# MarkTakken/kf2vecFSW

Hardware: AMD Instinct MI355X
Metric: Gbases/s k-mer→.kf build at k=7; achieved HBM GB/s vs gfx950 peak (higher is better)
Workload: dtype u32

## Files before the change

kf2vecfsw_amd/csrc/kf_bucket.hip:

```cpp
#include <hip/hip_runtime.h>
#include <stdint.h>
#include <stdlib.h>

#include <algorithm>
#include <cstdio>
#include <mutex>
#include <vector>

#include "kf_front.h"
#include "kf_internal.h"

namespace kf {


constexpr int kBkWaves = 16;
constexpr int kBkBits = 15;
constexpr uint64_t kPieceMax = (8ull << 20) - (64ull << 10);
constexpr uint32_t kBkLagShift = 3;
constexpr uint32_t kBkSlots = 2;
constexpr uint32_t kBkRoundWeights = 0x060B1114;
constexpr int kBkGroupWindows = 4;
constexpr bool bk_pre2(int K) { return K <= 10; }
constexpr uint32_t bk_rl(int K) { return K == 10 ? 4 : 0; }

// ... 858 lines not shown
        double sum[8] = {0, 0, 0, 0, 0, 0, 0, 0};
        for (int i = 0; i < grid; ++i)
            for (int x = 0; x < 8; ++x) sum[x] += (double)prof_h[8 * i + x];
        const double np = sum[2] > 0 ? sum[2] : 1;
        int occ = 0;
        (void)hipOccupancyMaxActiveBlocksPerMultiprocessor(&occ, (const void*)fn, waves * kWave, lds);
        fprintf(stderr, "[kf_bucket k=%d] grid %d x %d waves, LDS %u B, resident workgroups per CU %d\n", k, grid,
                waves, lds, occ);
        fprintf(stderr, "[kf_bucket k=%d] pieces %.0f cycles/piece: phase1 %.3g phase2 %.3g "
                "(records %.3g, barrier %.3g, flush %.3g, barrier %.3g)\n",
                k, sum[2], sum[0] / np, sum[1] / np, sum[3] / np, sum[4] / np, sum[5] / np, sum[6] / np);
        fprintf(stderr, "[kf_bucket k=%d] per wave, cycles per piece:", k);
        for (int w = 0; w < waves; ++w) {
            double v[4] = {0, 0, 0, 0};
            for (int i = 0; i < grid; ++i)
                for (int x = 0; x < 4; ++x) v[x] += (double)prof_h[8 * grid + 4 * (waves * i + w) + x];
            fprintf(stderr, "\n  w%d records %.3g (consume %.3g) barrier %.3g | phase-1 barrier %.3g", w, v[0] / np,
                    v[3] / np, v[1] / np, v[2] / np);
        }
        fprintf(stderr, "\n");
    }
    return KF_OK;
}

}

extern "C" int kf_workspace_release(void) {
    int dev = 0;
    if (hipGetDevice(&dev) != hipSuccess) return kf_fail(KF_EHIP, "hipGetDevice failed");
    if (dev < 0 || dev >= 64) return kf_fail(KF_EINVAL, "device index out of range");
    std::lock_guard<std::mutex> lk(g_mu);
    DevState& d = g_dev[dev];
    if (hipDeviceSynchronize() != hipSuccess) return kf_fail(KF_EHIP, "hipDeviceSynchronize failed");
    for (int k = 0; k <= KF_MAX_K; ++k) {
        if (d.col_idx[k]) (void)hipFree(d.col_idx[k]);
        if (d.bcol[k]) (void)hipFree(d.bcol[k]);
        d.col_idx[k] = nullptr;
        d.bcol[k] = nullptr;
    }
    if (d.scratch) (void)hipFree(d.scratch);
    if (d.pstart) (void)hipFree(d.pstart);
    d.scratch = nullptr;
    d.scratch_bytes = 0;
    d.pstart = nullptr;
    d.pstart_n = 0;
    return KF_OK;
}
```

kf2vecfsw_amd/csrc/kf_count.hip:

```cpp
#include <hip/hip_runtime.h>
#include <stdint.h>
#include <stdlib.h>

#include <mutex>

#include "kf_front.h"
#include "kf_internal.h"

namespace kf {

constexpr int kBlock = 1024;
constexpr uint32_t kWaveWeights = 20u | 17u << 8 | 11u << 16 | 6u << 24;
constexpr int kXRing = 2;

__device__ __forceinline__ void wg_span(const CountArgs& A, uint64_t& lo, uint64_t& hi) {
    const uint64_t base = A.goff[0];
    const uint64_t total = A.goff[A.n_genomes] - base;
    const uint64_t G = gridDim.x, b = blockIdx.x;
    lo = base + ((total / G * b + (total % G) * b / G) & ~(uint64_t)15);
    hi = (b + 1 == G) ? base + total : base + ((total / G * (b + 1) + (total % G) * (b + 1) / G) & ~(uint64_t)15);
}

template <int K>
struct XL {
    static constexpr uint32_t P = K >= 8 ? (1u << 17) : (2u << (2 * (K + 1)));
    static constexpr uint32_t S = K >= 8 ? (1u << 15) : (2u << (2 * K));
    static constexpr uint32_t bytes = P + S;
};
constexpr int kXChunk = 3 * kChunk;
static_assert((uint32_t)kXChunk == kLattice, "wave ranges are split on the iteration lattice (split_at_lattice)");
constexpr uint32_t kLatticeMaxIters = 2560;
constexpr uint32_t kHot7 = 0xC000C000u, kStep7 = 0x4000u;
constexpr uint32_t kHot8 = 0xE000E000u, kStep8 = 0x2000u;
constexpr uint32_t kHot6 = 0x80008000u, kStep6 = 0x8000u;
template <int K>
constexpr uint32_t x_hot() { return K >= 8 ? kHot8 : (K == 7 ? kHot7 : kHot6); }
template <int K>
constexpr uint32_t x_step() { return K >= 8 ? kStep8 : (K == 7 ? kStep7 : kStep6); }

__device__ __forceinline__ uint32_t k9_code_of(uint32_t i) { return ((i >> 9) << 10) | (i & 0x1FFu); }

__device__ __forceinline__ uint32_t half_one(uint32_t i) { return 1u << ((i & 1u) << 4); }

template <int B>
__device__ __forceinline__ uint32_t shl1_byte(uint32_t h, uint32_t one) {
    uint32_t r;
    if constexpr (B == 0)
        asm("v_lshlrev_b32_sdwa %0, %1, %2 dst_sel:DWORD dst_unused:UNUSED_PAD src0_sel:BYTE_0 src1_sel:DWORD"
            : "=v"(r) : "v"(h), "v"(one));
    else if constexpr (B == 1)
        asm("v_lshlrev_b32_sdwa %0, %1, %2 dst_sel:DWORD dst_unused:UNUSED_PAD src0_sel:BYTE_1 src1_sel:DWORD"
            : "=v"(r) : "v"(h), "v"(one));
    else if constexpr (B == 2)
        asm("v_lshlrev_b32_sdwa %0, %1, %2 dst_sel:DWORD dst_unused:UNUSED_PAD src0_sel:BYTE_2 src1_sel:DWORD"
            : "=v"(r) : "v"(h), "v"(one));
    else
        asm("v_lshlrev_b32_sdwa %0, %1, %2 dst_sel:DWORD dst_unused:UNUSED_PAD src0_sel:BYTE_3 src1_sel:DWORD"
            : "=v"(r) : "v"(h), "v"(one));
    return r;
}

// ... 32 lines not shown
    for (uint32_t w = (uint32_t)lane; w < (K >= 8 ? XL<K>::P : XL<K>::bytes) / 4; w += kWave) {
        const uint32_t v = __hip_atomic_load((lds_u32*)(uintptr_t)(4 * w), __ATOMIC_RELAXED,
                                             __HIP_MEMORY_SCOPE_WORKGROUP);
        if (v & HOT) x_drain<K>(4 * w, code2col, gcounts);
    }
}

constexpr uint32_t kXTabLo = 0x630B6102u;
constexpr uint32_t kXTabHi = 0x67000074u;

struct XBlock {
    uint4 q[3];
};
__device__ __forceinline__ uint32_t x_zmap(uint32_t x, uint32_t e, uint32_t c) {
    uint32_t r;
    asm("v_bitop3_b32 %0, %1, %2, %3 bitop3:0x38" : "=v"(r) : "v"(x), "v"(e), "v"(c));
    return r;
}

constexpr int kXNt = 2;

__device__ __forceinline__ XBlock xc_load(const uint8_t* bytes, uint64_t c0, uint32_t rel, uint32_t end_r, int lane) {
    const uint32_t rec = end_r > rel ? min(end_r - rel, (uint32_t)kXChunk) : 0u;
    const auto rs = __builtin_amdgcn_make_buffer_rsrc((void*)(bytes + c0 + rel), (short)0, (int)rec, 0x00020000);
    XBlock b;
#pragma unroll
    for (int i = 0; i < 3; ++i) {
        const auto v = __builtin_amdgcn_raw_buffer_load_b128(rs, lane * 16 + kChunk * i, 0, kXNt);
        b.q[i] = make_uint4(v[0], v[1], v[2], v[3]);
    }
    return b;
}

__device__ __forceinline__ constexpr uint32_t xc_nl_weights(int i) {
    return (uint32_t)(64 - 8 * i) | (uint32_t)(62 - 8 * i) << 8 | (uint32_t)(60 - 8 * i) << 16 |
           (uint32_t)(58 - 8 * i) << 24;
}
constexpr uint32_t kXcBad = 68u;

struct XcCls {
    uint32_t C, V;
};
__device__ __forceinline__ XcCls xc_cls(const uint4 d) {
    const uint32_t w[4] = {d.x, d.y, d.z, d.w};
    const uint32_t cdf = 0xDFDFDFDFu;
    uint32_t pc[4], z[4];
#pragma unroll
    for (int i = 0; i < 4; ++i) {
        const uint32_t x = w[i];
        const uint32_t e = __builtin_amdgcn_perm(kXTabHi, kXTabLo, x & 0x07070707u);
        z[i] = x_zmap(x, e, cdf);
        pc[i] = __builtin_amdgcn_udot4(x & 0x06060606u, 0x01041040u, (i & 1) ? pc[i - 1] << 8 : 0u, false);
    }
    XcCls r;
    r.C = (pc[1] << 15) | (pc[3] >> 1);
    r.V = __builtin_amdgcn_udot4(z[1], xc_nl_weights(1), __builtin_amdgcn_udot4(z[0], xc_nl_weights(0), 0u, false),
                                 false) +
          __builtin_amdgcn_udot4(z[3], xc_nl_weights(3), __builtin_amdgcn_udot4(z[2], xc_nl_weights(2), 0u, false),
                                 false);
    return r;
}

struct XcWin {
    uint32_t x0, y0, c, nl;
};
__device__ __forceinline__ XcWin xc_window(const XcCls& k, uint32_t rot) {
// ... 184 lines not shown

template <int K, bool MASKED>
__device__ __forceinline__ uint32_t x_singles(const uint4 d, const CountArgs& A, uint64_t chunk, int lane,
                                              const ChunkMask& m, uint64_t iv0, uint32_t carry, uint32_t* gcounts,
                                              uint32_t& lane_total, uint32_t& drained) {
    constexpr uint32_t HOT = x_hot<K>();
    uint32_t C, V, EN, ne, own;
    front_end<K, MASKED, false>(d, A, chunk, lane, m, iv0, C, V, EN, ne, own);
    const Windows win = windows<K, MASKED>(C, V, EN, ne, carry, lane);
    const uint32_t wlo = win.wlo, whi = win.whi, R = win.R;
    if constexpr (K == 9) {
        drained |= k9b_region<false>(wlo, whi, R, A, gcounts);
        lane_total += (uint32_t)__builtin_popcount(R);
        return win.next;
    }
    const uint32_t wv[4] = {wlo, __builtin_amdgcn_alignbit(whi, wlo, 8), __builtin_amdgcn_alignbit(whi, wlo, 16),
                            __builtin_amdgcn_alignbit(whi, wlo, 24)};
    uint32_t o = 0;
#pragma unroll
    for (int r = 0; r < 16; ++r) {
        const int fo = (2 * r) & ~7;
        const uint32_t y = __builtin_amdgcn_ubfe(wv[fo >> 3], 2 * r - fo, 2 * K);
        o |= lds_add_rtn((K == 8 ? 0u : XL<K>::P) + ((y >> 1) << 2), ((R >> r) & 1u) * half_one(y));
    }
    if (__builtin_amdgcn_ballot_w64((o & HOT) != 0) != 0) {
        x_scan_drain<K>(A.code2col, gcounts, lane);
        drained = 1;
    }
    lane_total += (uint32_t)__builtin_popcount(R);
    return win.next;
}

template <int K>
__device__ __forceinline__ uint32_t x_range(const CountArgs& A, int32_t g, uint64_t glo, uint64_t ghi, uint64_t lo,
                                            uint64_t hi, int lane, uint64_t& iv_hint, uint32_t& drained) {
    if (lo >= hi) return 0;
    uint32_t* gcounts = A.counts + (uint64_t)g * A.nbins;
    Range rg;
    rg.init(glo, ghi, lo, hi);
    auto load = [&](uint32_t r) {
        return xc_load(A.bytes, rg.c0, r, rg.end_r, lane);
    };
    static_assert(kXRing == 2, "two-deep register ring");
    XBlock buf[K == 9 ? 1 : kXRing];
    XBlock b0, b1;
    if constexpr (K == 9) {
        b0 = load(0);
        b1 = load(kXChunk);
    } else {
#pragma unroll
        for (int j = 0; j < kXRing; ++j) buf[j] = load(j * kXChunk);
    }
    const uint32_t nx = (rg.nch + 2) / 3;
    rg.warm16<K>(A, lane, iv_hint);
    __builtin_amdgcn_s_setprio(0);
    uint32_t carry = rg.carry;
    uint32_t rel = 0;
    const ChunkMask m = rg.mask();
    uint32_t lane_total = 0;
    uint32_t nfast = 0;
    auto step = [&](const XBlock& bf) {
        bool fast = !rg.masked_span(A, rel, kXChunk);
        if (fast)
            fast = xc_fast<K>(bf, A, lane, carry, gcounts, lane_total, drained);
        nfast += fast ? 1u : 0u;
        if (!fast) {
            const bool m0 = rg.masked(A, rel);
            const uint64_t iv0 = rg.iv;
            const bool m1 = rg.masked(A, rel + kChunk);
            const uint64_t iv1 = rg.iv;
// ... 50 lines not shown
#pragma unroll
        for (int a = 0; a < 4; ++a) {
            const uint32_t v = hist[a * 8192 + i * 1024 + tid];
            F[2 * i] += v & 0xFFFFu;
            F[2 * i + 1] += v >> 16;
        }
    }
}

template <int K>
__device__ __forceinline__ void pair_f_sums_small(const uint32_t* hist, int tid,
                                                  uint32_t (&F)[((1u << (2 * K)) + kBlock - 1) / kBlock]) {
    constexpr uint32_t NY = 1u << (2 * K), NM = (NY + kBlock - 1) / kBlock;
#pragma unroll
    for (uint32_t m = 0; m < NM; ++m) {
        const uint32_t y = (uint32_t)tid + kBlock * m;
        F[m] = 0;
        if (y < NY) {
            const uint32_t sh = (y & 1u) << 4;
            uint32_t f = u16sum2(hist[2 * y]) + u16sum2(hist[2 * y + 1]);
#pragma unroll
            for (uint32_t a = 0; a < 4; ++a) f += (hist[a * (NY / 2) + (y >> 1)] >> sh) & 0xFFFFu;
            f += (hist[XL<K>::P / 4 + (y >> 1)] >> sh) & 0xFFFFu;
            F[m] = f;
        }
    }
}

__device__ __forceinline__ void lds_zero(uint32_t* hist, uint32_t lo4, uint32_t hi4, int tid) {
    uint4* h4 = (uint4*)hist;
    for (uint32_t i = lo4 + (uint32_t)tid; i < hi4; i += kBlock) h4[i] = make_uint4(0u, 0u, 0u, 0u);
}

template <int K>
__global__ void __launch_bounds__(kBlock) __attribute__((amdgpu_waves_per_eu(4, 4))) k1x_kernel(CountArgs A) {
    static_assert(K >= 2 && K <= 9, "K1x serves k = 2 .. 9 (k = 9: K9b byte counters)");
    extern __shared__ __attribute__((aligned(16))) uint32_t hist[];
    const int tid = threadIdx.x;
    const int lane = tid & (kWave - 1);
    const int wave = __builtin_amdgcn_readfirstlane(tid >> 6);
    {
        uint4* h4 = (uint4*)hist;
        for (uint32_t i = tid; i < XL<K>::bytes / 16; i += kBlock) h4[i] = make_uint4(0u, 0u, 0u, 0u);
    }
    __syncthreads();
    if ((uint32_t)(uintptr_t)(lds_u32*)hist != 0u) __builtin_trap();
    uint64_t span_lo, span_hi;
    wg_span(A, span_lo, span_hi);
    if (span_lo >= span_hi) return;
    int32_t g = (int32_t)wave_upper_bound((uint64_t)A.n_genomes, span_lo, lane,
                                          [&](uint64_t i) { return A.goff[i + 1]; });
    const uint32_t fr_lo = wave_frac((uint32_t)wave, kWaveWeights), fr_hi = wave_frac((uint32_t)wave + 1, kWaveWeights);
    uint64_t g_lo = A.goff[g], g_hi = A.goff[g + 1];
    uint64_t iv_hint = 0;
    for (; g < A.n_genomes; ++g) {
        __builtin_amdgcn_s_setprio(3);
        const uint64_t glo = g_lo, ghi = g_hi;
        g_lo = g_hi;
        g_hi = A.goff[min(g + 2, A.n_genomes)];
        if (glo >= span_hi) break;
        const uint64_t plo = max(glo, span_lo), phi = min(ghi, span_hi);
        if (phi <= plo) continue;
        const uint32_t nit = lattice_iters(plo, phi);
        const bool lat = nit <= kLatticeMaxIters;
        const uint64_t lo = split_at_lattice(plo, phi, nit, lat, fr_lo), hi = split_at_lattice(plo, phi, nit, lat, fr_hi);
        uint32_t drained = 0;
        unsigned long long s = x_range<K>(A, g, glo, ghi, lo, hi, lane, iv_hint, drained);
        uint32_t* gc = A.counts + (uint64_t)g * A.nbins;
        const bool whole = plo == glo && phi == ghi && !(A.flags & KF_ACCUMULATE);
        if constexpr (K == 9) {
            lds_barrier();
            if (lane == 0) hist[XL<K>::P / 4 + wave] = drained;
            lds_barrier();
            const uint4* fl = (const uint4*)(hist + XL<K>::P / 4);
            const uint4 f0 = fl[0], f1 = fl[1], f2 = fl[2], f3 = fl[3];
            const bool any_fix = (f0.x | f0.y | f0.z | f0.w | f1.x | f1.y | f1.z | f1.w | f2.x | f2.y | f2.z |
                                  f2.w | f3.x | f3.y | f3.z | f3.w) != 0;
            const uint8_t* hb = (const uint8_t*)hist;
            for (uint32_t c0 = (uint32_t)tid; c0 < (1u << 17); c0 += 4 * kBlock) {
                uint32_t rep[4];
#pragma unroll
                for (int j = 0; j < 4; ++j) rep[j] = A.col2rep[c0 + j * kBlock];
#pragma unroll
                for (int j = 0; j < 4; ++j) {
                    const uint32_t c = (rep[j] & 0x200u) ? kf_revcomp<9>(rep[j]) : rep[j];
                    const uint32_t v = hb[((c >> 1) & 0x1FE00u) | (c & 0x1FFu)];
                    if (whole && !any_fix)
                        __builtin_nontemporal_store(v, gc + c0 + j * kBlock);
                    else if (v)
                        __hip_atomic_fetch_add(gc + c0 + j * kBlock, v, __ATOMIC_RELAXED, __HIP_MEMORY_SCOPE_AGENT);
                }
            }
            lds_barrier();
            uint4* h4 = (uint4*)hist;
            for (uint32_t i = tid; i < XL<K>::bytes / 16; i += kBlock) h4[i] = make_uint4(0u, 0u, 0u, 0u);
        } else if constexpr (K == 8) {
            lds_barrier();
            if (lane == 0) hist[XL<K>::P / 4 + wave] = drained;
            lds_barrier();
            const uint4* fl = (const uint4*)(hist + XL<K>::P / 4);
            const uint4 f0 = fl[0], f1 = fl[1], f2 = fl[2], f3 = fl[3];
            const bool any_drain = (f0.x | f0.y | f0.z | f0.w | f1.x | f1.y | f1.z | f1.w | f2.x | f2.y | f2.z |
                                    f2.w | f3.x | f3.y | f3.z | f3.w) != 0;
            for (uint32_t col = tid; col < A.nbins; col += kBlock) {
                const uint32_t y = A.col2rep[col], rc = kf_revcomp<8>(y);
                uint32_t v = (hist[y >> 1] >> ((y & 1u) << 4)) & 0xFFFFu;
                if (rc != y) v += (hist[rc >> 1] >> ((rc & 1u) << 4)) & 0xFFFFu;
                if (whole && !any_drain)
                    gc[col] = v;
                else if (v)
                    __hip_atomic_fetch_add(gc + col, v, __ATOMIC_RELAXED, __HIP_MEMORY_SCOPE_AGENT);
            }
            lds_barrier();
            uint4* h4 = (uint4*)hist;
            for (uint32_t i = tid; i < XL<K>::bytes / 16; i += kBlock) h4[i] = make_uint4(0u, 0u, 0u, 0u);
        } else if constexpr (K <= 6) {
            constexpr uint32_t NY = 1u << (2 * K), NM = (NY + kBlock - 1) / kBlock;
            constexpr uint32_t NCOL = (NY + (K % 2 == 0 ? (1u << K) : 0u)) / 2, NC = (NCOL + kBlock - 1) / kBlock;
            constexpr uint32_t ZF = (NY + 16) / 4;
            static_assert(ZF <= XL<K>::bytes / 16, "F and the flags lie inside the table");
            uint32_t rep[NC];
#pragma unroll
            for (uint32_t c = 0; c < NC; ++c) {
                const uint32_t col = (uint32_t)tid + c * kBlock;
                rep[c] = col < NCOL ? A.col2rep[col] : 0u;
            }
            lds_barrier();
            uint32_t F[NM];
            pair_f_sums_small<K>(hist, tid, F);
            lds_barrier();
#pragma unroll
            for (uint32_t m = 0; m < NM; ++m) {
                const uint32_t y = (uint32_t)tid + kBlock * m;
                if (y < NY) hist[f_swz(y)] = F[m];
            }
            if (lane == 0) hist[NY + wave] = drained;
            lds_zero(hist, ZF, XL<K>::bytes / 16, tid);
            lds_barrier();
            const uint4* fl = (const uint4*)(hist + NY);
            const uint4 f0 = fl[0], f1 = fl[1], f2 = fl[2], f3 = fl[3];
            const bool any_drain = (f0.x | f0.y | f0.z | f0.w | f1.x | f1.y | f1.z | f1.w | f2.x | f2.y | f2.z | f2.w |
                                    f3.x | f3.y | f3.z | f3.w) != 0;
            uint32_t cv[NC];
#pragma unroll
            for (uint32_t c = 0; c < NC; ++c) {
                const uint32_t y = rep[c], rc = kf_revcomp<K>(y);
                cv[c] = hist[f_swz(y)] + (rc != y ? hist[f_swz(rc)] : 0u);
            }
            lds_barrier();
            lds_zero(hist, 0, ZF, tid);
#pragma unroll
            for (uint32_t c = 0; c < NC; ++c) {
                const uint32_t col = (uint32_t)tid + c * kBlock;
                if (col >= NCOL) continue;
                if (whole && !any_drain)
                    __builtin_nontemporal_store(cv[c], gc + col);
                else if (cv[c])
                    __hip_atomic_fetch_add(gc + col, cv[c], __ATOMIC_RELAXED, __HIP_MEMORY_SCOPE_AGENT);
            }
        } else {
            uint32_t rep[8];
            if (whole) {
                const uint4 r0 = *(const uint4*)(A.col2rep + 4 * tid), r1 = *(const uint4*)(A.col2rep + 4096 + 4 * tid);
                rep[0] = r0.x, rep[1] = r0.y, rep[2] = r0.z, rep[3] = r0.w;
                rep[4] = r1.x, rep[5] = r1.y, rep[6] = r1.z, rep[7] = r1.w;
            } else {
#pragma unroll
                for (int c = 0; c < 8; ++c) rep[c] = A.col2rep[tid + c * kBlock];
            }
            lds_barrier();
            uint32_t F[16];
            pair_f_sums(hist, tid, F);
#pragma unroll
            for (int i = 0; i < 8; ++i) {
                const uint32_t v = hist[XL<K>::P / 4 + i * 1024 + tid];
                F[2 * i] += v & 0xFFFFu;
                F[2 * i + 1] += v >> 16;
            }
            lds_barrier();
#pragma unroll
            for (int i = 0; i < 8; ++i) *(uint2*)(hist + f_swz(i * 2048 + 2 * tid)) = make_uint2(F[2 * i], F[2 * i + 1]);
            if (lane == 0) hist[16384 + wave] = drained;
            constexpr uint32_t ZF = (16384 + 16) / 4;
            lds_zero(hist, ZF, XL<K>::bytes / 16, tid);
            lds_barrier();
            const uint4* fl = (const uint4*)(hist + 16384);
            const uint4 f0 = fl[0], f1 = fl[1], f2 = fl[2], f3 = fl[3];
            const bool any_drain = (f0.x | f0.y | f0.z | f0.w | f1.x | f1.y | f1.z | f1.w | f2.x | f2.y | f2.z | f2.w |
                                    f3.x | f3.y | f3.z | f3.w) != 0;
            uint32_t cv[8];
#pragma unroll
            for (int c = 0; c < 8; ++c) {
                const uint32_t y = rep[c], rc = kf_revcomp<7>(y);
                cv[c] = hist[f_swz(y)] + hist[f_swz(rc)];
            }
            lds_barrier();
            lds_zero(hist, 0, ZF, tid);
            if (whole && !any_drain) {
                typedef unsigned int v4u_t __attribute__((ext_vector_type(4)));
                __builtin_nontemporal_store(v4u_t{cv[0], cv[1], cv[2], cv[3]}, (v4u_t*)(gc + 4 * tid));
                __builtin_nontemporal_store(v4u_t{cv[4], cv[5], cv[6], cv[7]}, (v4u_t*)(gc + 4096 + 4 * tid));
            } else {
#pragma unroll
                for (int c = 0; c < 8; ++c) {
                    const uint32_t col = whole ? (c >> 2) * 4096 + 4 * tid + (c & 3) : tid + c * kBlock;
                    if (cv[c]) __hip_atomic_fetch_add(gc + col, cv[c], __ATOMIC_RELAXED, __HIP_MEMORY_SCOPE_AGENT);
                }
            }
        }
        s = wave_sum(s);
        if (lane == 0 && s) atomicAdd(A.totals + g, s);
        lds_barrier();
    }
}

__device__ __forceinline__ uint64_t splitmix64(uint64_t x) {
    x += 0x9E3779B97F4A7C15ull;
    x = (x ^ (x >> 30)) * 0xBF58476D1CE4E5B9ull;
    x = (x ^ (x >> 27)) * 0x94D049BB133111EBull;
    return x ^ (x >> 31);
}

__device__ __forceinline__ bool in_nrun(uint64_t key, uint64_t i, uint64_t n_period) {
    if (!n_period) return false;
    uint64_t b = i >> 12;
    for (int d = 0; d < 2; ++d) {
        if (d == 1) {
            if (b == 0) break;
            b -= 1;
        }
        const uint64_t h = splitmix64((key ^ 0xA5A5A5A5A5A5A5A5ull) + b);
        if (h % n_period) continue;
        const uint64_t st = (b << 12) + ((h >> 16) % 4096), ln = 1 + ((h >> 32) % 100);
        if (i >= st && i < st + ln) return true;
    }
    return false;
}

__global__ void __launch_bounds__(256) synth_kernel(uint8_t* bytes, const uint64_t* goff, int64_t g0, int64_t gstride,
                                                     uint64_t seed0, uint64_t seq_len, int width, uint64_t n_period) {
    const int32_t gi = blockIdx.y;
    const uint64_t lo = goff[gi], hi = goff[gi + 1];
    const int64_t g = g0 + gi * gstride;
    char digits[24];
    int nd = 0;
// ... 77 lines not shown

using namespace kf;

namespace {

void* kernel_for(int k) {
    switch (k) {
    case 2: return (void*)&k1x_kernel<2>;
    case 3: return (void*)&k1x_kernel<3>;
    case 4: return (void*)&k1x_kernel<4>;
    case 5: return (void*)&k1x_kernel<5>;
    case 6: return (void*)&k1x_kernel<6>;
    case 7: return (void*)&k1x_kernel<7>;
    case 8: return (void*)&k1x_kernel<8>;
    case 9: return (void*)&k1x_kernel<9>;
    default: return nullptr;
    }
}

int lds_bytes_for(int k) {
    switch (k) {
    case 2: return (int)XL<2>::bytes;
    case 3: return (int)XL<3>::bytes;
    case 4: return (int)XL<4>::bytes;
    case 5: return (int)XL<5>::bytes;
    case 6: return (int)XL<6>::bytes;
    case 7: return (int)XL<7>::bytes;
    case 8: return (int)XL<8>::bytes;
    default: return (int)XL<9>::bytes;
    }
}


int g_grid[KF_MAX_K + 1][64];
std::mutex g_grid_mu;

int launch_info(int k, int* grid, int* block, int* lds) {
    int dev = 0;
    if (hipGetDevice(&dev) != hipSuccess) return kf_fail(KF_EHIP, "hipGetDevice failed");
    if (dev < 0 || dev >= 64) return kf_fail(KF_EINVAL, "device index out of range");
    const int l = lds_bytes_for(k);
    std::lock_guard<std::mutex> lk(g_grid_mu);
    int& gr = g_grid[k][dev];
    if (!gr) {
        void* fn = kernel_for(k);
        if (hipFuncSetAttribute(fn, hipFuncAttributeMaxDynamicSharedMemorySize, l) != hipSuccess)
            return kf_fail(KF_EHIP, "hipFuncSetAttribute(MaxDynamicSharedMemorySize) failed");
        int per_cu = 0, cus = 0;
        if (hipOccupancyMaxActiveBlocksPerMultiprocessor(&per_cu, fn, kBlock, l) != hipSuccess)
            return kf_fail(KF_EHIP, "hipOccupancyMaxActiveBlocksPerMultiprocessor failed");
        if (hipDeviceGetAttribute(&cus, hipDeviceAttributeMultiprocessorCount, dev) != hipSuccess)
            return kf_fail(KF_EHIP, "hipDeviceGetAttribute(MultiprocessorCount) failed");
        gr = (per_cu < 1 ? 1 : per_cu) * (cus > 0 ? cus : 1);
    }
    *grid = gr;
    *block = kBlock;
    *lds = l;
    return KF_OK;
}
}

extern "C" int kf_count_launch_info(int k, int* grid, int* block, int* lds_bytes) {
    if (k < KF_MIN_K || k > KF_MAX_K) return kf_fail(KF_EINVAL, "k out of range [2, 12]");
    if (!grid || !block || !lds_bytes) return kf_fail(KF_EINVAL, "null output pointer");
    if (k >= 10) return bucket_launch_info(k, grid, block, lds_bytes);
    return launch_info(k, grid, block, lds_bytes);
}

extern "C" int kf_workspace_reserve(int k, int32_t max_genomes) {
    if (k < KF_MIN_K || k > KF_MAX_K) return kf_fail(KF_EINVAL, "k out of range [2, 12]");
    if (max_genomes < 0) return kf_fail(KF_EINVAL, "max_genomes < 0");
    if (k >= 10) return bucket_reserve(k, max_genomes);
    int grid = 0, block = 0, lds = 0;
    return launch_info(k, &grid, &block, &lds);
}

extern "C" int kf_count_batch(const uint8_t* d_bytes, const uint64_t* d_goff, int32_t n_genomes,
                              const uint64_t* d_excl, uint64_t n_excl, const uint32_t* d_code2col,
                              const uint32_t* d_col2rep, int k, uint32_t* d_counts, uint64_t* d_totals,
                              uint32_t flags, void* stream) {
    if (k < KF_MIN_K || k > KF_MAX_K) return kf_fail(KF_EINVAL, "k out of range [2, 12]");
    if (n_genomes < 0) return kf_fail(KF_EINVAL, "n_genomes < 0");
    if (n_genomes == 0) return KF_OK;
    if (!d_bytes || !d_goff || !d_counts || !d_totals || !d_code2col || !d_col2rep)
        return kf_fail(KF_EINVAL, "null device pointer");
    if (n_excl && !d_excl) return kf_fail(KF_EINVAL, "d_excl is null but n_excl > 0");
    if (((uintptr_t)d_bytes) & 15) return kf_fail(KF_EINVAL, "d_bytes must be 16-byte aligned");
    const uint64_t nb = kf_num_bins(k);
    hipStream_t s = (hipStream_t)stream;
    const bool bucket = k >= 10;
    if (!(flags & KF_ACCUMULATE)) {
        if ((!bucket && hipMemsetAsync(d_counts, 0, (size_t)n_genomes * nb * sizeof(uint32_t), s) != hipSuccess) ||
            hipMemsetAsync(d_totals, 0, (size_t)n_genomes * sizeof(uint64_t), s) != hipSuccess)
            return kf_fail(KF_EHIP, "hipMemsetAsync failed");
    }
    CountArgs A;
    A.bytes = d_bytes;
    A.goff = d_goff;
    A.excl = d_excl;
    A.n_excl = n_excl;
    A.code2col = d_code2col;
    A.col2rep = d_col2rep;
    A.counts = d_counts;
    A.totals = (unsigned long long*)d_totals;
    A.nbins = (uint32_t)nb;
    A.n_genomes = n_genomes;
    A.flags = flags;
    if (bucket) return bucket_launch(A, k, flags, s);
    int grid = 0, block = 0, lds = 0;
    const int rc = launch_info(k, &grid, &block, &lds);
    if (rc) return rc;

    void* args[] = {&A};
    if (hipLaunchKernel(kernel_for(k), dim3(grid), dim3(block), args, (size_t)lds, s) != hipSuccess)
        return kf_fail(KF_EHIP, "count kernel launch failed: %s", hipGetErrorString(hipGetLastError()));
    return KF_OK;
}

extern "C" int kf_stream_probe(const uint8_t* d_bytes, uint64_t n, uint32_t* d_out, void* stream) {
    if (!d_bytes || !d_out) return kf_fail(KF_EINVAL, "null device pointer");
    if (((uintptr_t)d_bytes) & 15) return kf_fail(KF_EINVAL, "d_bytes must be 16-byte aligned");
    if (n == 0) return KF_OK;
    int dev = 0, cus = 0;
    if (hipGetDevice(&dev) != hipSuccess ||
        hipDeviceGetAttribute(&cus, hipDeviceAttributeMultiprocessorCount, dev) != hipSuccess)
        return kf_fail(KF_EHIP, "device query failed");
    hipLaunchKernelGGL(stream_probe_kernel, dim3(2 * (cus > 0 ? cus : 1)), dim3(1024), 0, (hipStream_t)stream, d_bytes,
                       n, d_out);
    if (hipGetLastError() != hipSuccess) return kf_fail(KF_EHIP, "stream probe launch failed");
    return KF_OK;
}

extern "C" int kf_synth_fasta(uint8_t* d_bytes, const uint64_t* d_goff, int32_t n_genomes, int64_t g0,
                              int64_t g_stride, uint64_t seed0, uint64_t seq_len, int width, uint64_t n_period,
                              void* stream) {
    if (n_genomes <= 0) return n_genomes == 0 ? KF_OK : kf_fail(KF_EINVAL, "n_genomes < 0");
    if (!d_bytes || !d_goff) return kf_fail(KF_EINVAL, "null device pointer");
    if (width < 1) return kf_fail(KF_EINVAL, "width < 1");
    if (n_genomes > 65535) return kf_fail(KF_EINVAL, "at most 65535 genomes per synth call");
    dim3 grid(512, (unsigned)n_genomes);
    hipLaunchKernelGGL(synth_kernel, grid, dim3(256), 0, (hipStream_t)stream, d_bytes, d_goff, g0, g_stride, seed0,
                       seq_len, width, n_period);
    if (hipGetLastError() != hipSuccess) return kf_fail(KF_EHIP, "synth kernel launch failed");
    return KF_OK;
}
```

kf2vecfsw_amd/csrc/kf_front.h:

```cpp
#pragma once
#include <hip/hip_runtime.h>
#include <stdint.h>

#include "kf_scan.h"

namespace kf {

constexpr int kWave = 64;
constexpr int kChunk = 1024;

struct CountArgs {
    const uint8_t* bytes;
    const uint64_t* goff;
    const uint64_t* excl;
    uint64_t n_excl;
    const uint32_t* code2col;
    const uint32_t* col2rep;
    uint32_t* counts;
    unsigned long long* totals;
    uint32_t nbins;
    int32_t n_genomes;
    uint32_t flags;
};

// ... 409 lines not shown
};
template <int K, bool MASKED>
__device__ __forceinline__ Windows windows(uint32_t C, uint32_t V, uint32_t EN, uint32_t ne, uint32_t carry,
                                           int lane) {
    constexpr uint32_t TM = (K > 1) ? ((1u << (2 * (K - 1))) - 1u) : 0u;
    const uint32_t own = own_tail<K>(C, V, ne);
    uint32_t ctx = wave_shr1(carry, own);
    if (__ballot(ne < (uint32_t)(K - 1)) != 0) {
        const uint64_t inc_mask = __ballot(!tail_complete<K>(own)) & 0x7FFFFFFFFFFFFFFFull;
        if (inc_mask) ctx = scan_ctx<K>(own, carry, lane);
    }
    const uint64_t W = ((uint64_t)t_codes(ctx) << (2 * ne)) | (uint64_t)C;
    Windows w;
    w.wlo = (uint32_t)W;
    w.whi = (uint32_t)(W >> 32);
    const uint32_t ctxlen = min(t_n(ctx), (uint32_t)(K - 1));
    const uint32_t E = (((1u << ctxlen) - 1u) << ne) | V;
    w.R = run_mask<K>(E) & ((1u << ne) - 1u);
    if (MASKED) w.R &= EN;
    const uint32_t incl = tail_pack(w.wlo & TM, (uint32_t)__builtin_ctz(~E), 31u);
    w.next = (uint32_t)__builtin_amdgcn_readlane((int)incl, kWave - 1);
    return w;
}

__device__ __forceinline__ unsigned long long wave_sum(unsigned long long v) {
#pragma unroll
    for (int d = 32; d >= 1; d >>= 1) v += __shfl_xor(v, d, kWave);
    return v;
}

int bucket_launch(const CountArgs& A, int k, uint32_t flags, hipStream_t s);
int bucket_launch_info(int k, int* grid, int* block, int* lds);
int bucket_reserve(int k, int32_t max_genomes);

}
```

Measured before the change: 6124.

## Replace count/totals memsets with per-block scratch rows and in-kernel totals

Removes the full hipMemsetAsync of the counts matrix and totals for k<=9. A small prepare kernel now zeroes only empty genomes and genomes split across block boundaries. Blocks that own a whole genome drain overflow into a per-block scratch row, then write the final counts and totals directly; split genomes still use atomics. It also touches the next genome's leading cache lines early. This adds a second launch, persistent scratch allocation, cross-stream event ordering, and more complex correctness invariants.

```diff
diff --git a/kf2vecfsw_amd/csrc/kf_bucket.hip b/kf2vecfsw_amd/csrc/kf_bucket.hip
--- a/kf2vecfsw_amd/csrc/kf_bucket.hip
+++ b/kf2vecfsw_amd/csrc/kf_bucket.hip
@@ -914,6 +914,7 @@
     std::lock_guard<std::mutex> lk(g_mu);
     DevState& d = g_dev[dev];
     if (hipDeviceSynchronize() != hipSuccess) return kf_fail(KF_EHIP, "hipDeviceSynchronize failed");
+    kf::count_release(dev);
     for (int k = 0; k <= KF_MAX_K; ++k) {
         if (d.col_idx[k]) (void)hipFree(d.col_idx[k]);
         if (d.bcol[k]) (void)hipFree(d.bcol[k]);
diff --git a/kf2vecfsw_amd/csrc/kf_count.hip b/kf2vecfsw_amd/csrc/kf_count.hip
--- a/kf2vecfsw_amd/csrc/kf_count.hip
+++ b/kf2vecfsw_amd/csrc/kf_count.hip
@@ -13,20 +13,25 @@
 constexpr uint32_t kWaveWeights = 20u | 17u << 8 | 11u << 16 | 6u << 24;
 constexpr int kXRing = 2;
 
+__device__ __forceinline__ uint64_t span_cut(uint64_t base, uint64_t total, uint64_t G, uint64_t b) {
+    return b >= G ? base + total : base + ((total / G * b + (total % G) * b / G) & ~(uint64_t)15);
+}
 __device__ __forceinline__ void wg_span(const CountArgs& A, uint64_t& lo, uint64_t& hi) {
     const uint64_t base = A.goff[0];
     const uint64_t total = A.goff[A.n_genomes] - base;
-    const uint64_t G = gridDim.x, b = blockIdx.x;
-    lo = base + ((total / G * b + (total % G) * b / G) & ~(uint64_t)15);
-    hi = (b + 1 == G) ? base + total : base + ((total / G * (b + 1) + (total % G) * (b + 1) / G) & ~(uint64_t)15);
+    lo = span_cut(base, total, gridDim.x, blockIdx.x);
+    hi = span_cut(base, total, gridDim.x, (uint64_t)blockIdx.x + 1);
 }
 
 template <int K>
 struct XL {
     static constexpr uint32_t P = K >= 8 ? (1u << 17) : (2u << (2 * (K + 1)));
     static constexpr uint32_t S = K >= 8 ? (1u << 15) : (2u << (2 * K));
-    static constexpr uint32_t bytes = P + S;
+    static constexpr uint32_t flush = K <= 6 ? 4u * ((1u << (2 * K)) + 48u) : 0u;
+    static constexpr uint32_t bytes = P + S > flush ? P + S : flush;
 };
+constexpr uint32_t kFlushWords = 16 + 2 * 16;
+static_assert(XL<2>::flush == 4u * (16u + kFlushWords), "XL::flush holds kFlushWords");
 constexpr int kXChunk = 3 * kChunk;
 static_assert((uint32_t)kXChunk == kLattice, "wave ranges are split on the iteration lattice (split_at_lattice)");
 constexpr uint32_t kLatticeMaxIters = 2560;
@@ -125,6 +130,13 @@
     return b;
 }
 
+__device__ __forceinline__ uint32_t touch_lines(const uint8_t* bytes, uint64_t at, uint64_t end, int lane) {
+    const uint64_t a0 = at & ~(uint64_t)127, s0 = a0 >= 128 ? a0 - 128 : 0, e = (end + 15) & ~(uint64_t)15;
+    const uint32_t rec = e > s0 ? (uint32_t)min(e - s0, (uint64_t)8192) : 0u;
+    const auto rs = __builtin_amdgcn_make_buffer_rsrc((void*)(bytes + s0), (short)0, (int)rec, 0x00020000);
+    return (uint32_t)__builtin_amdgcn_raw_buffer_load_b32(rs, lane * 128, 0, 0);
+}
+
 __device__ __forceinline__ constexpr uint32_t xc_nl_weights(int i) {
     return (uint32_t)(64 - 8 * i) | (uint32_t)(62 - 8 * i) << 8 | (uint32_t)(60 - 8 * i) << 16 |
            (uint32_t)(58 - 8 * i) << 24;
@@ -375,10 +387,9 @@
 }
 
 template <int K>
-__device__ __forceinline__ uint32_t x_range(const CountArgs& A, int32_t g, uint64_t glo, uint64_t ghi, uint64_t lo,
-                                            uint64_t hi, int lane, uint64_t& iv_hint, uint32_t& drained) {
+__device__ __forceinline__ uint32_t x_range(const CountArgs& A, uint32_t* gcounts, uint64_t glo, uint64_t ghi,
+                                            uint64_t lo, uint64_t hi, int lane, uint64_t& iv_hint, uint32_t& drained) {
     if (lo >= hi) return 0;
-    uint32_t* gcounts = A.counts + (uint64_t)g * A.nbins;
     Range rg;
     rg.init(glo, ghi, lo, hi);
     auto load = [&](uint32_t r) {
@@ -495,8 +506,47 @@
     for (uint32_t i = lo4 + (uint32_t)tid; i < hi4; i += kBlock) h4[i] = make_uint4(0u, 0u, 0u, 0u);
 }
 
+__device__ __forceinline__ void flush_post(uint32_t* fw, int lane, int wave, uint32_t drained, unsigned long long s) {
+    if (lane == 0) {
+        fw[wave] = drained;
+        *(uint2*)(fw + 16 + 2 * wave) = make_uint2((uint32_t)s, (uint32_t)(s >> 32));
+    }
+}
+__device__ __forceinline__ bool flush_any(const uint32_t* fw) {
+    const uint4* fl = (const uint4*)fw;
+    const uint4 f0 = fl[0], f1 = fl[1], f2 = fl[2], f3 = fl[3];
+    return (f0.x | f0.y | f0.z | f0.w | f1.x | f1.y | f1.z | f1.w | f2.x | f2.y | f2.z | f2.w | f3.x | f3.y | f3.z |
+            f3.w) != 0;
+}
+__device__ __forceinline__ void flush_total(const uint32_t* fw, int lane, int wave, bool whole, unsigned long long s,
+                                            unsigned long long* total) {
+    if (whole) {
+        if (wave != 0) return;
+        const uint4* tw = (const uint4*)(fw + 16);
+        unsigned long long t = 0;
+#pragma unroll
+        for (int i = 0; i < 8; ++i) {
+            const uint4 w = tw[i];
+            t += ((unsigned long long)w.y << 32 | w.x) + ((unsigned long long)w.w << 32 | w.z);
+        }
+        if (lane == 0) *total = t;
+    } else if (lane == 0 && s) {
+        atomicAdd(total, s);
+    }
+}
+
+typedef __attribute__((address_space(1))) uint32_t global_u32;
+__device__ __forceinline__ uint32_t d_load(uint32_t* d) {
+    return __hip_atomic_load((global_u32*)(uintptr_t)d, __ATOMIC_RELAXED, __HIP_MEMORY_SCOPE_AGENT);
+}
+__device__ __forceinline__ void d_clear(uint32_t* d) {
+    __hip_atomic_store((global_u32*)(uintptr_t)d, 0u, __ATOMIC_RELAXED, __HIP_MEMORY_SCOPE_AGENT);
+}
+__device__ __forceinline__ void vmem_done() { __builtin_amdgcn_s_waitcnt(0x0F70); }
+
 template <int K>
-__global__ void __launch_bounds__(kBlock) __attribute__((amdgpu_waves_per_eu(4, 4))) k1x_kernel(CountArgs A) {
+__global__ void __launch_bounds__(kBlock) __attribute__((amdgpu_waves_per_eu(4, 4))) k1x_kernel(CountArgs A,
+                                                                                                 uint32_t* D) {
     static_assert(K >= 2 && K <= 9, "K1x serves k = 2 .. 9 (k = 9: K9b byte counters)");
     extern __shared__ __attribute__((aligned(16))) uint32_t hist[];
     const int tid = threadIdx.x;
@@ -527,18 +577,29 @@
         const uint32_t nit = lattice_iters(plo, phi);
         const bool lat = nit <= kLatticeMaxIters;
         const uint64_t lo = split_at_lattice(plo, phi, nit, lat, fr_lo), hi = split_at_lattice(plo, phi, nit, lat, fr_hi);
+        const bool whole = plo == glo && phi == ghi && !(A.flags & KF_ACCUMULATE);
+        uint32_t* gc = A.counts + (uint64_t)g * A.nbins;
+        auto scratch_row = [&]() {
+            uint32_t* p = D + (uint64_t)blockIdx.x * A.nbins;
+            asm volatile("" : "+s"(p));
+            return p;
+        };
         uint32_t drained = 0;
-        unsigned long long s = x_range<K>(A, g, glo, ghi, lo, hi, lane, iv_hint, drained);
-        uint32_t* gc = A.counts + (uint64_t)g * A.nbins;
-        const bool whole = plo == glo && phi == ghi && !(A.flags & KF_ACCUMULATE);
+        unsigned long long s = x_range<K>(A, whole ? scratch_row() : gc, glo, ghi, lo, hi, lane, iv_hint, drained);
+        s = wave_sum(s);
+        if (__builtin_amdgcn_readfirstlane(drained)) vmem_done();
+        uint32_t touched = 0;
+        if (const uint64_t nlo = g_lo, nhi = min(g_hi, span_hi); g + 1 < A.n_genomes && nlo < nhi) {
+            const uint32_t nn = lattice_iters(nlo, nhi);
+            touched = touch_lines(A.bytes, split_at_lattice(nlo, nhi, nn, nn <= kLatticeMaxIters, fr_lo), span_hi, lane);
+        }
         if constexpr (K == 9) {
             lds_barrier();
-            if (lane == 0) hist[XL<K>::P / 4 + wave] = drained;
-            lds_barrier();
-            const uint4* fl = (const uint4*)(hist + XL<K>::P / 4);
-            const uint4 f0 = fl[0], f1 = fl[1], f2 = fl[2], f3 = fl[3];
-            const bool any_fix = (f0.x | f0.y | f0.z | f0.w | f1.x | f1.y | f1.z | f1.w | f2.x | f2.y | f2.z |
-                                  f2.w | f3.x | f3.y | f3.z | f3.w) != 0;
+            uint32_t* fw = hist + XL<K>::P / 4;
+            flush_post(fw, lane, wave, drained, s);
+            lds_barrier();
+            const bool any_fix = flush_any(fw);
+            flush_total(fw, lane, wave, whole, s, A.totals + g);
             const uint8_t* hb = (const uint8_t*)hist;
             for (uint32_t c0 = (uint32_t)tid; c0 < (1u << 17); c0 += 4 * kBlock) {
                 uint32_t rep[4];
@@ -548,40 +609,51 @@
                 for (int j = 0; j < 4; ++j) {
                     const uint32_t c = (rep[j] & 0x200u) ? kf_revcomp<9>(rep[j]) : rep[j];
                     const uint32_t v = hb[((c >> 1) & 0x1FE00u) | (c & 0x1FFu)];
-                    if (whole && !any_fix)
+                    if (whole && !any_fix) {
                         __builtin_nontemporal_store(v, gc + c0 + j * kBlock);
-                    else if (v)
+                    } else if (whole) {
+                        uint32_t* drow = scratch_row();
+                        gc[c0 + j * kBlock] = v + d_load(drow + c0 + j * kBlock);
+                        d_clear(drow + c0 + j * kBlock);
+                    } else if (v) {
                         __hip_atomic_fetch_add(gc + c0 + j * kBlock, v, __ATOMIC_RELAXED, __HIP_MEMORY_SCOPE_AGENT);
+                    }
                 }
             }
+            if (whole && any_fix) vmem_done();
             lds_barrier();
             uint4* h4 = (uint4*)hist;
             for (uint32_t i = tid; i < XL<K>::bytes / 16; i += kBlock) h4[i] = make_uint4(0u, 0u, 0u, 0u);
         } else if constexpr (K == 8) {
             lds_barrier();
-            if (lane == 0) hist[XL<K>::P / 4 + wave] = drained;
-            lds_barrier();
-            const uint4* fl = (const uint4*)(hist + XL<K>::P / 4);
-            const uint4 f0 = fl[0], f1 = fl[1], f2 = fl[2], f3 = fl[3];
-            const bool any_drain = (f0.x | f0.y | f0.z | f0.w | f1.x | f1.y | f1.z | f1.w | f2.x | f2.y | f2.z |
-                                    f2.w | f3.x | f3.y | f3.z | f3.w) != 0;
+            uint32_t* fw = hist + XL<K>::P / 4;
+            flush_post(fw, lane, wave, drained, s);
+            lds_barrier();
+            const bool any_drain = flush_any(fw);
+            flush_total(fw, lane, wave, whole, s, A.totals + g);
             for (uint32_t col = tid; col < A.nbins; col += kBlock) {
                 const uint32_t y = A.col2rep[col], rc = kf_revcomp<8>(y);
                 uint32_t v = (hist[y >> 1] >> ((y & 1u) << 4)) & 0xFFFFu;
                 if (rc != y) v += (hist[rc >> 1] >> ((rc & 1u) << 4)) & 0xFFFFu;
-                if (whole && !any_drain)
+                if (whole && !any_drain) {
                     gc[col] = v;
-                else if (v)
+                } else if (whole) {
+                    uint32_t* drow = scratch_row();
+                    gc[col] = v + d_load(drow + col);
+                    d_clear(drow + col);
+                } else if (v) {
                     __hip_atomic_fetch_add(gc + col, v, __ATOMIC_RELAXED, __HIP_MEMORY_SCOPE_AGENT);
-            }
+                }
+            }
+            if (whole && any_drain) vmem_done();
             lds_barrier();
             uint4* h4 = (uint4*)hist;
             for (uint32_t i = tid; i < XL<K>::bytes / 16; i += kBlock) h4[i] = make_uint4(0u, 0u, 0u, 0u);
         } else if constexpr (K <= 6) {
             constexpr uint32_t NY = 1u << (2 * K), NM = (NY + kBlock - 1) / kBlock;
             constexpr uint32_t NCOL = (NY + (K % 2 == 0 ? (1u << K) : 0u)) / 2, NC = (NCOL + kBlock - 1) / kBlock;
-            constexpr uint32_t ZF = (NY + 16) / 4;
-            static_assert(ZF <= XL<K>::bytes / 16, "F and the flags lie inside the table");
+            constexpr uint32_t ZF = (NY + kFlushWords) / 4;
+            static_assert(ZF <= XL<K>::bytes / 16, "F, the flags and the totals lie inside the table");
             uint32_t rep[NC];
 #pragma unroll
             for (uint32_t c = 0; c < NC; ++c) {
@@ -597,13 +669,11 @@
                 const uint32_t y = (uint32_t)tid + kBlock * m;
                 if (y < NY) hist[f_swz(y)] = F[m];
             }
-            if (lane == 0) hist[NY + wave] = drained;
+            flush_post(hist + NY, lane, wave, drained, s);
             lds_zero(hist, ZF, XL<K>::bytes / 16, tid);
             lds_barrier();
-            const uint4* fl = (const uint4*)(hist + NY);
-            const uint4 f0 = fl[0], f1 = fl[1], f2 = fl[2], f3 = fl[3];
-            const bool any_drain = (f0.x | f0.y | f0.z | f0.w | f1.x | f1.y | f1.z | f1.w | f2.x | f2.y | f2.z | f2.w |
-                                    f3.x | f3.y | f3.z | f3.w) != 0;
+            const bool any_drain = flush_any(hist + NY);
+            flush_total(hist + NY, lane, wave, whole, s, A.totals + g);
             uint32_t cv[NC];
 #pragma unroll
             for (uint32_t c = 0; c < NC; ++c) {
@@ -616,11 +686,17 @@
             for (uint32_t c = 0; c < NC; ++c) {
                 const uint32_t col = (uint32_t)tid + c * kBlock;
                 if (col >= NCOL) continue;
-                if (whole && !any_drain)
+                if (whole && !any_drain) {
                     __builtin_nontemporal_store(cv[c], gc + col);
-                else if (cv[c])
+                } else if (whole) {
+                    uint32_t* drow = scratch_row();
+                    gc[col] = cv[c] + d_load(drow + col);
+                    d_clear(drow + col);
+                } else if (cv[c]) {
                     __hip_atomic_fetch_add(gc + col, cv[c], __ATOMIC_RELAXED, __HIP_MEMORY_SCOPE_AGENT);
-            }
+                }
+            }
+            if (whole && any_drain) vmem_done();
         } else {
             uint32_t rep[8];
             if (whole) {
@@ -643,14 +719,12 @@
             lds_barrier();
 #pragma unroll
             for (int i = 0; i < 8; ++i) *(uint2*)(hist + f_swz(i * 2048 + 2 * tid)) = make_uint2(F[2 * i], F[2 * i + 1]);
-            if (lane == 0) hist[16384 + wave] = drained;
-            constexpr uint32_t ZF = (16384 + 16) / 4;
+            flush_post(hist + 16384, lane, wave, drained, s);
+            constexpr uint32_t ZF = (16384 + kFlushWords) / 4;
             lds_zero(hist, ZF, XL<K>::bytes / 16, tid);
             lds_barrier();
-            const uint4* fl = (const uint4*)(hist + 16384);
-            const uint4 f0 = fl[0], f1 = fl[1], f2 = fl[2], f3 = fl[3];
-            const bool any_drain = (f0.x | f0.y | f0.z | f0.w | f1.x | f1.y | f1.z | f1.w | f2.x | f2.y | f2.z | f2.w |
-                                    f3.x | f3.y | f3.z | f3.w) != 0;
+            const bool any_drain = flush_any(hist + 16384);
+            flush_total(hist + 16384, lane, wave, whole, s, A.totals + g);
             uint32_t cv[8];
 #pragma unroll
             for (int c = 0; c < 8; ++c) {
@@ -663,17 +737,53 @@
                 typedef unsigned int v4u_t __attribute__((ext_vector_type(4)));
                 __builtin_nontemporal_store(v4u_t{cv[0], cv[1], cv[2], cv[3]}, (v4u_t*)(gc + 4 * tid));
                 __builtin_nontemporal_store(v4u_t{cv[4], cv[5], cv[6], cv[7]}, (v4u_t*)(gc + 4096 + 4 * tid));
+            } else if (whole) {
+                uint32_t* drow = scratch_row();
+#pragma unroll
+                for (int c = 0; c < 8; ++c) {
+                    const uint32_t col = (c >> 2) * 4096 + 4 * tid + (c & 3);
+                    gc[col] = cv[c] + d_load(drow + col);
+                    d_clear(drow + col);
+                }
+                vmem_done();
             } else {
 #pragma unroll
                 for (int c = 0; c < 8; ++c) {
-                    const uint32_t col = whole ? (c >> 2) * 4096 + 4 * tid + (c & 3) : tid + c * kBlock;
+                    const uint32_t col = tid + c * kBlock;
                     if (cv[c]) __hip_atomic_fetch_add(gc + col, cv[c], __ATOMIC_RELAXED, __HIP_MEMORY_SCOPE_AGENT);
                 }
             }
         }
-        s = wave_sum(s);
-        if (lane == 0 && s) atomicAdd(A.totals + g, s);
+        asm volatile("" ::"v"(touched));
         lds_barrier();
+    }
+}
+
+__device__ __forceinline__ void zero_genome(const CountArgs& A, uint64_t g, uint32_t t, uint32_t nthr) {
+    uint32_t* row = A.counts + g * A.nbins;
+    if ((A.nbins & 3u) == 0 && ((uintptr_t)A.counts & 15) == 0) {
+        for (uint32_t i = t; i < A.nbins / 4; i += nthr) ((uint4*)row)[i] = make_uint4(0u, 0u, 0u, 0u);
+    } else {
+        for (uint32_t i = t; i < A.nbins; i += nthr) row[i] = 0u;
+    }
+    if (t == 0) A.totals[g] = 0ull;
+}
+
+__global__ void __launch_bounds__(256) prepare_kernel(CountArgs A, uint32_t G) {
+    const uint32_t tid = threadIdx.x, lane = tid & (kWave - 1);
+    const uint64_t n = (uint64_t)A.n_genomes;
+    for (uint64_t g0 = ((uint64_t)blockIdx.x * blockDim.x + tid) & ~(uint64_t)(kWave - 1); g0 < n;
+         g0 += (uint64_t)gridDim.x * blockDim.x) {
+        const uint64_t g = g0 + lane;
+        uint64_t m = __builtin_amdgcn_ballot_w64(g < n && A.goff[g] == A.goff[g + 1]);
+        for (; m; m &= m - 1) zero_genome(A, g0 + (uint64_t)__builtin_ctzll(m), lane, kWave);
+    }
+    for (uint32_t b = blockIdx.x; b < G; b += gridDim.x) {
+        if (b == 0) continue;
+        const uint64_t base = A.goff[0];
+        const uint64_t cut = span_cut(base, A.goff[n] - base, G, b);
+        const uint64_t g = wave_upper_bound(n, cut, (int)lane, [&](uint64_t i) { return A.goff[i + 1]; });
+        if (g < n && A.goff[g] < cut) zero_genome(A, g, tid, blockDim.x);
     }
 }
 
@@ -817,31 +927,77 @@
 }
 
 
-int g_grid[KF_MAX_K + 1][64];
+struct CountDev {
+    int grid[KF_MAX_K + 1] = {};
+    uint32_t* D[KF_MAX_K + 1] = {};
+    hipEvent_t done = nullptr;
+    hipStream_t last = nullptr;
+    bool used = false;
+};
+CountDev g_cdev[64];
 std::mutex g_grid_mu;
 
-int launch_info(int k, int* grid, int* block, int* lds) {
-    int dev = 0;
-    if (hipGetDevice(&dev) != hipSuccess) return kf_fail(KF_EHIP, "hipGetDevice failed");
-    if (dev < 0 || dev >= 64) return kf_fail(KF_EINVAL, "device index out of range");
+int current_device(int* dev) {
+    if (hipGetDevice(dev) != hipSuccess) return kf_fail(KF_EHIP, "hipGetDevice failed");
+    if (*dev < 0 || *dev >= 64) return kf_fail(KF_EINVAL, "device index out of range");
+    return KF_OK;
+}
+
+int ensure_rows(CountDev& cd, int k) {
+    if (cd.D[k]) return KF_OK;
+    const size_t bytes = (size_t)cd.grid[k] * kf_num_bins(k) * sizeof(uint32_t);
+    if (!cd.done && hipEventCreateWithFlags(&cd.done, hipEventDisableTiming) != hipSuccess)
+        return kf_fail(KF_EHIP, "hipEventCreate failed");
+    uint32_t* p = nullptr;
+    if (hipMalloc((void**)&p, bytes) != hipSuccess)
+        return kf_fail(KF_EHIP, "hipMalloc of %zu bytes of count scratch rows failed", bytes);
+    if (hipMemset(p, 0, bytes) != hipSuccess || hipDeviceSynchronize() != hipSuccess) {
+        (void)hipFree(p);
+        return kf_fail(KF_EHIP, "zeroing the count scratch rows failed");
+    }
+    cd.D[k] = p;
+    return KF_OK;
+}
+
+int order_rows(CountDev& cd, hipStream_t s) {
+    if (cd.used && cd.last != s) {
+        if (hipEventRecord(cd.done, cd.last) != hipSuccess) {
+            (void)hipGetLastError();
+            if (hipDeviceSynchronize() != hipSuccess) return kf_fail(KF_EHIP, "hipDeviceSynchronize failed");
+        } else if (hipStreamWaitEvent(s, cd.done, 0) != hipSuccess) {
+            return kf_fail(KF_EHIP, "hipStreamWaitEvent failed");
+        }
+    }
+    cd.last = s;
+    cd.used = true;
+    return KF_OK;
+}
+
+int ensure_grid(CountDev& cd, int dev, int k) {
+    if (cd.grid[k]) return KF_OK;
     const int l = lds_bytes_for(k);
+    void* fn = kernel_for(k);
+    if (hipFuncSetAttribute(fn, hipFuncAttributeMaxDynamicSharedMemorySize, l) != hipSuccess)
+        return kf_fail(KF_EHIP, "hipFuncSetAttribute(MaxDynamicSharedMemorySize) failed");
+    int per_cu = 0, cus = 0;
+    if (hipOccupancyMaxActiveBlocksPerMultiprocessor(&per_cu, fn, kBlock, l) != hipSuccess)
+        return kf_fail(KF_EHIP, "hipOccupancyMaxActiveBlocksPerMultiprocessor failed");
+    if (hipDeviceGetAttribute(&cus, hipDeviceAttributeMultiprocessorCount, dev) != hipSuccess)
+        return kf_fail(KF_EHIP, "hipDeviceGetAttribute(MultiprocessorCount) failed");
+    cd.grid[k] = (per_cu < 1 ? 1 : per_cu) * (cus > 0 ? cus : 1);
+    return KF_OK;
+}
+}
+
+namespace kf {
+void count_release(int dev) {
     std::lock_guard<std::mutex> lk(g_grid_mu);
-    int& gr = g_grid[k][dev];
-    if (!gr) {
-        void* fn = kernel_for(k);
-        if (hipFuncSetAttribute(fn, hipFuncAttributeMaxDynamicSharedMemorySize, l) != hipSuccess)
-            return kf_fail(KF_EHIP, "hipFuncSetAttribute(MaxDynamicSharedMemorySize) failed");
-        int per_cu = 0, cus = 0;
-        if (hipOccupancyMaxActiveBlocksPerMultiprocessor(&per_cu, fn, kBlock, l) != hipSuccess)
-            return kf_fail(KF_EHIP, "hipOccupancyMaxActiveBlocksPerMultiprocessor failed");
-        if (hipDeviceGetAttribute(&cus, hipDeviceAttributeMultiprocessorCount, dev) != hipSuccess)
-            return kf_fail(KF_EHIP, "hipDeviceGetAttribute(MultiprocessorCount) failed");
-        gr = (per_cu < 1 ? 1 : per_cu) * (cus > 0 ? cus : 1);
-    }
-    *grid = gr;
-    *block = kBlock;
-    *lds = l;
-    return KF_OK;
+    CountDev& cd = g_cdev[dev];
+    for (int k = 0; k <= KF_MAX_K; ++k) {
+        if (cd.D[k]) (void)hipFree(cd.D[k]);
+        cd.D[k] = nullptr;
+    }
+    cd.used = false;
 }
 }
 
@@ -849,15 +1005,28 @@
     if (k < KF_MIN_K || k > KF_MAX_K) return kf_fail(KF_EINVAL, "k out of range [2, 12]");
     if (!grid || !block || !lds_bytes) return kf_fail(KF_EINVAL, "null output pointer");
     if (k >= 10) return bucket_launch_info(k, grid, block, lds_bytes);
-    return launch_info(k, grid, block, lds_bytes);
+    int dev = 0;
+    int rc = current_device(&dev);
+    if (rc) return rc;
+    std::lock_guard<std::mutex> lk(g_grid_mu);
+    rc = ensure_grid(g_cdev[dev], dev, k);
+    if (rc) return rc;
+    *grid = g_cdev[dev].grid[k];
+    *block = kBlock;
+    *lds_bytes = lds_bytes_for(k);
+    return KF_OK;
 }
 
 extern "C" int kf_workspace_reserve(int k, int32_t max_genomes) {
     if (k < KF_MIN_K || k > KF_MAX_K) return kf_fail(KF_EINVAL, "k out of range [2, 12]");
     if (max_genomes < 0) return kf_fail(KF_EINVAL, "max_genomes < 0");
     if (k >= 10) return bucket_reserve(k, max_genomes);
-    int grid = 0, block = 0, lds = 0;
-    return launch_info(k, &grid, &block, &lds);
+    int dev = 0;
+    int rc = current_device(&dev);
+    if (rc) return rc;
+    std::lock_guard<std::mutex> lk(g_grid_mu);
+    rc = ensure_grid(g_cdev[dev], dev, k);
+    return rc ? rc : ensure_rows(g_cdev[dev], k);
 }
 
 extern "C" int kf_count_batch(const uint8_t* d_bytes, const uint64_t* d_goff, int32_t n_genomes,
@@ -874,11 +1043,9 @@
     const uint64_t nb = kf_num_bins(k);
     hipStream_t s = (hipStream_t)stream;
     const bool bucket = k >= 10;
-    if (!(flags & KF_ACCUMULATE)) {
-        if ((!bucket && hipMemsetAsync(d_counts, 0, (size_t)n_genomes * nb * sizeof(uint32_t), s) != hipSuccess) ||
-            hipMemsetAsync(d_totals, 0, (size_t)n_genomes * sizeof(uint64_t), s) != hipSuccess)
-            return kf_fail(KF_EHIP, "hipMemsetAsync failed");
-    }
+    const bool accumulate = (flags & KF_ACCUMULATE) != 0;
+    if (bucket && !accumulate && hipMemsetAsync(d_totals, 0, (size_t)n_genomes * sizeof(uint64_t), s) != hipSuccess)
+        return kf_fail(KF_EHIP, "hipMemsetAsync failed");
     CountArgs A;
     A.bytes = d_bytes;
     A.goff = d_goff;
@@ -892,12 +1059,25 @@
     A.n_genomes = n_genomes;
     A.flags = flags;
     if (bucket) return bucket_launch(A, k, flags, s);
-    int grid = 0, block = 0, lds = 0;
-    const int rc = launch_info(k, &grid, &block, &lds);
+    int dev = 0;
+    int rc = current_device(&dev);
     if (rc) return rc;
-
-    void* args[] = {&A};
-    if (hipLaunchKernel(kernel_for(k), dim3(grid), dim3(block), args, (size_t)lds, s) != hipSuccess)
+    std::lock_guard<std::mutex> lk(g_grid_mu);
+    CountDev& cd = g_cdev[dev];
+    rc = ensure_grid(cd, dev, k);
+    if (rc) return rc;
+    const uint32_t grid = (uint32_t)cd.grid[k];
+    uint32_t* D = nullptr;
+    if (!accumulate) {
+        rc = ensure_rows(cd, k);
+        if (!rc) rc = order_rows(cd, s);
+        if (rc) return rc;
+        D = cd.D[k];
+        hipLaunchKernelGGL(prepare_kernel, dim3(grid), dim3(256), 0, s, A, grid);
+        if (hipGetLastError() != hipSuccess) return kf_fail(KF_EHIP, "prepare kernel launch failed");
+    }
+    void* args[] = {&A, &D};
+    if (hipLaunchKernel(kernel_for(k), dim3(grid), dim3(kBlock), args, (size_t)lds_bytes_for(k), s) != hipSuccess)
         return kf_fail(KF_EHIP, "count kernel launch failed: %s", hipGetErrorString(hipGetLastError()));
     return KF_OK;
 }
diff --git a/kf2vecfsw_amd/csrc/kf_front.h b/kf2vecfsw_amd/csrc/kf_front.h
--- a/kf2vecfsw_amd/csrc/kf_front.h
+++ b/kf2vecfsw_amd/csrc/kf_front.h
@@ -465,5 +465,6 @@
 int bucket_launch(const CountArgs& A, int k, uint32_t flags, hipStream_t s);
 int bucket_launch_info(int k, int* grid, int* block, int* lds);
 int bucket_reserve(int k, int32_t max_genomes);
-
-}
+void count_release(int dev);
+
+}
```

Result: no change. 6120 (-0.1%).
